# vinits5/bullet-envs

Measured on AMD Instinct MI355X. Metric: env-steps/sec (whole node), 16-link snake, 4096 envs/GPU, higher is better.
Workload: dtype f32

## Files before the change

### bullet-envs_amd/csrc/snk_pgs_v2.hpp

```cpp
#pragma once
#include "snk_contacts.hpp"
#include "snk_dynamics.hpp"
#include "snk_lds.hpp"
#include "snk_model.hpp"
#include "snk_selfcol.hpp"
#include "snk_wave.hpp"

namespace snk {


constexpr int kSlotNormal = 0;
constexpr int kSlotFric = 32;
constexpr int kSlots = 96;
constexpr int kAppMotor = 0;
constexpr int kAppNormal = 16;
constexpr int kAppFric = 80;
constexpr unsigned long long kLowMask = 0x00000000FFFFFFFFull;


struct ObsHit {
    bool hit;
    f3 P, n, dA, dB;
    float dist;
};
// ... 215 lines not shown
        f3 P = mk3(0, 0, 0), d = mk3(0, 0, 0);
        float* Mrow = motor ? L.Mm[mj] : L.stM[lane];
        if (motor) {
            k = mj + 1;
        } else {
            k = L.ccbody[ci];
            P = ld3(L.ccP[ci]);
            d = NORMAL ? (ci < L.nplane ? mk3(0.f, 0.f, 1.f) : ld3(L.obn[ci - L.nplane])) : ld3(L.cdir[L.ccds[ci]][lane >> 5]);
        }
        f3 pN = mk3(0, 0, 0), pF = mk3(0, 0, 0);
        const f3 oK = ld3(L.o[motor ? 0 : k]);
        BodyK cur = load_body_k(L, N);
#pragma unroll 4
        for (int b = N; b >= 1; b--) {
            const BodyK nxt = load_body_k(L, b > 1 ? b - 1 : 1);
            f3 ax = cur.ax;
            if (!motor && b == k) {
                pN = pN - cross(P - oK, d);
                pF = pF - d;
            }
            float u = -dot(ax, pN);
            if (motor && b == k) u += 1.0f;
            Mrow[6 + b - 1] = u;
            float t = u * cur.Dinv;
            f3 paN = pN + cur.Ua * t, paF = pF + cur.Ub * t;
            pN = paN + cross(cur.r, paF);
            pF = paF;
            cur = nxt;
        }
        f3 J0 = mk3(0, 0, 0), J1 = mk3(0, 0, 0);
        if (!motor) {
            J0 = cross(P - ld3(L.o[0]), d);
            J1 = d;
            if (k == 0) { pN = pN - J0; pF = pF - d; }
        }
        float p0[6] = {pN.x, pN.y, pN.z, pF.x, pF.y, pF.z}, a0[6];
#pragma unroll
        for (int i = 0; i < 6; i++) {
            float sum = 0.f;
#pragma unroll
            for (int j = 0; j < 6; j++) sum -= L.Inv0[6 * i + j] * p0[j];
            a0[i] = sum;
            Mrow[i] = sum;
        }
        f3 al = mk3(a0[0], a0[1], a0[2]), a = mk3(a0[3], a0[4], a0[5]);
        const float* gb = L.base() + 7;
        float den = dot(J0, al) + dot(J1, a);
        float rv = dot(J0, ld3(gb)) + dot(J1, ld3(gb + 3));
        cur = load_body_k(L, 1);
        f3 ob = ld3(L.o[1]);
        float qdb = L.qd()[0], ub = Mrow[6];
#pragma unroll 4
        for (int b = 1; b <= N; b++) {
            const int bn = b < N ? b + 1 : N;
            const BodyK nxt = load_body_k(L, bn);
            const f3 obn = ld3(L.o[bn]);
            const float qdn = L.qd()[bn - 1], un = Mrow[6 + bn - 1];
            a = a + cross(al, cur.r);
            float u = ub;
            float qdd = (u - (dot(cur.Ua, al) + dot(cur.Ub, a))) * cur.Dinv;
            f3 ax = cur.ax;
            al = al + ax * qdd;
            Mrow[6 + b - 1] = qdd;
            if (!motor) {
                float Jb = (b <= k) ? dot(ax, cross(P - ob, d)) : 0.f;
                den += Jb * qdd;
                rv += Jb * qdb;
            } else if (b == k) {
                den = qdd;
            }
            cur = nxt; ob = obn; qdb = qdn; ub = un;
        }
        float dinv = den > 1.1920929e-7f ? 1.0f / den : 0.f;
        float target;
        if (motor) {
            float cur = L.qd()[mj];
            float want = M.kp * (L.targets[mj] - L.q()[mj]) * M.inv_dt + cur + M.kd * (0.f - cur);
            target = want - cur;
        } else if (NORMAL) {
            float pen = L.ccdist[lane] + M.slop;
            float erp = M.contact_erp;
            if constexpr (LT::kERP) erp = pen > M.erp_split ? M.erp_shallow : M.erp_deep;
            target = -rv + (pen > 0.f ? -pen * M.inv_dt : -pen * erp * M.inv_dt);
        } else {
            target = -rv;
        }
        float* S = motor ? L.MmS[mj] : &L.stM[lane][22];
        S[0] = target * dinv;
        S[1] = den;
        S[2] = dinv;
        if (motor) S[3] = target;
    }
    lds_sync();
}


struct LaneK {
    int h, d;
    bool isdof;
    float m22, m24;
    float m31;
    int spoff;
    f3 oL, aL;
    int bL;
};

struct SlotRaw {
    float mval, dinv, sp, lam;
    f3 P, dir;
    int k;
    bool valid;
};
template <class LT, int KIND>
__device__ __forceinline__ SlotRaw fetch_slot(LT& L, const LaneK& K, int s, int count, int base, int nplane) {
    SlotRaw r;
    const int ci = KIND == 1 ? 2 * s + K.h : s;
    r.valid = ci < count;
    const int rs = r.valid ? ci : 0;
    const int row = KIND == 1 ? rs : (r.valid ? 32 * K.h + (s - base) : 0);
    const float* st = L.stM[row];
    const int dd = K.isdof ? K.d : 0;
    r.mval = st[dd];
    r.dinv = st[24];
    r.sp = st[22 + K.spoff];
    r.P = ld3(L.ccP[rs]);
    r.dir = KIND == 1 ? (rs < nplane ? mk3(0.f, 0.f, 1.f) : ld3(L.obn[rs - nplane])) : ld3(L.cdir[L.ccds[rs]][K.h]);
    r.k = L.ccbody[rs];
    r.lam = (KIND == 1 && r.valid) ? L.app[kAppNormal + rs] : 0.f;
    return r;
}
template <int KIND>
__device__ __forceinline__ void finish_slot(const SlotRaw& r, const LaneK& K, float sJ, float sM, float& RJ, float& RM,
                                            float& wsum) {
    float v = dot(K.aL, cross(r.P - K.oL, r.dir));
    v = K.d == 3 ? r.dir.x : (K.d == 4 ? r.dir.y : (K.d == 5 ? r.dir.z : v));
    const float jd = (K.bL <= r.k) ? v : 0.0f;
    float rj = (K.isdof ? jd * r.dinv : r.sp * K.m22) * sJ;
    float rm = (K.isdof ? r.mval : r.sp * K.m24) * sM;
    if (!r.valid) { rj = 0.f; rm = 0.f; }
    if (KIND == 1) {
        rj += K.m31 * r.lam;
        wsum += rm * r.lam;
    }
    RJ = rj;
    RM = rm;
}
struct MuScale {
    float fJ, fM, fJo, fMo;
    int nplane;
};
template <class LT, int KIND, int BASE, int DST>
__device__ __forceinline__ void load_slots8(LT& L, const LaneK& K, int count, int base, const MuScale& ms,
                                            float (&RJ)[kSlots], float (&RM)[kSlots], float& wsum) {
    SlotRaw cur = fetch_slot<LT, KIND>(L, K, BASE, count, base, ms.nplane);
#pragma unroll
    for (int i = 0; i < 8; i++) {
        SlotRaw nxt = cur;
        if (i < 7) nxt = fetch_slot<LT, KIND>(L, K, BASE + i + 1, count, base, ms.nplane);
        const bool gr = KIND == 1 || BASE + i < ms.nplane;
        finish_slot<KIND>(cur, K, KIND == 1 ? 1.0f : (gr ? ms.fJ : ms.fJo), KIND == 1 ? 1.0f : (gr ? ms.fM : ms.fMo),
                          RJ[DST + BASE + i], RM[DST + BASE + i], wsum);
        cur = nxt;
    }
}

#define SNK_REDUCE_12 \
    "v_add_f32_dpp %[t], %[t], %[t] quad_perm:[1,0,3,2] row_mask:0xf bank_mask:0xf bound_ctrl:1\n\t"
#define SNK_REDUCE_22 \
    "v_add_f32_dpp %[t], %[t], %[t] quad_perm:[2,3,0,1] row_mask:0xf bank_mask:0xf bound_ctrl:1\n\t"
#define SNK_REDUCE_345                                                                            \
    "v_add_f32_dpp %[t], %[t], %[t] row_shr:4 row_mask:0xf bank_mask:0xf bound_ctrl:1\n\t"         \
    "s_nop 1\n\t"                                                                                  \
    "v_add_f32_dpp %[t], %[t], %[t] row_shr:8 row_mask:0xf bank_mask:0xf bound_ctrl:1\n\t"         \
    "s_nop 1\n\t"                                                                                  \
    "v_add_f32_dpp %[t], %[t], %[t] row_bcast:15 row_mask:0xa bank_mask:0xf\n\t"                   \
    "s_nop 0\n\t"

#define SNK_DUO_HEAD                                     \
    "v_mul_f32 %[t], %[RJ], %[dv]\n\t"                    \
    "v_readlane_b32 %[s2], %[RJ], 31\n\t"                 \
    "v_readlane_b32 %[s3], %[RJ], 63\n\t"                 \
    SNK_REDUCE_12                                          \
    "s_nop 1\n\t"                                         \
    SNK_REDUCE_22                                          \
    "s_nop 1\n\t"                                         \
    SNK_REDUCE_345                                         \
    "v_readlane_b32 %[s0], %[t], 31\n\t"                  \
    "s_nop 1\n\t"
#define SNK_ACC3163(RJ_, T_) "v_add_f32_dpp " RJ_ ", " T_ ", " RJ_ " row_shr:15 row_mask:0xa bank_mask:0xf\n\t"
#define SNK_DUO_TAIL                                     \
    "v_cndmask_b32_e64 %[t], %[dS], %[dF], %[lowmask]\n\t" \
    "v_mul_f32 %[x], %[RM], %[t]\n\t"                     \
    "v_mul_f32 %[c2], %[RM], %[t]\n\t"                    \
    SNK_ACC3163("%[RJ]", "%[t]")                           \
    "s_nop 0\n\t"                                         \
    "v_permlane32_swap_b32 %[x], %[c2]\n\t"               \
    "v_add_f32 %[dv], %[dv], %[x]\n\t"                    \
    "v_add_f32 %[dv], %[dv], %[c2]\n\t"
template <bool RES, bool BOX>
__device__ __forceinline__ void duo_step(float& RJ, const float RM, float& dv, float HI, float E3163,
                                         unsigned long long lowmask, float& lsq) {
    float t, x, dF, dS, c2;
    float s0, s1, s2, s3;
    if (!BOX) {
        asm volatile(
            SNK_DUO_HEAD
            "v_max_f32_e64 %[dF], -%[s0], 0\n\t"
            "v_subrev_f32 %[dF], %[s2], %[dF]\n\t"
            "s_nop 0\n\t"
            "v_fmac_f32_dpp %[t], %[RJ], %[dF] row_shr:1 row_mask:0xf bank_mask:0xf bound_ctrl:1\n\t"
            "s_nop 0\n\t"
            "v_readlane_b32 %[s1], %[t], 63\n\t"
            "s_nop 1\n\t"
            "v_max_f32_e64 %[x], -%[s1], 0\n\t"
            "v_subrev_f32 %[dS], %[s3], %[x]\n\t"
            SNK_DUO_TAIL
            : [t] "=&v"(t), [x] "=&v"(x), [dF] "=&v"(dF), [dS] "=&v"(dS), [c2] "=&v"(c2), [s0] "=&s"(s0), [s1] "=&s"(s1),
              [s2] "=&s"(s2), [s3] "=&s"(s3), [RJ] "+v"(RJ), [dv] "+v"(dv)
            : [RM] "v"(RM), [lowmask] "s"(lowmask));
    } else
    asm volatile(
        SNK_DUO_HEAD
        "v_med3_f32 %[dF], -%[s0], -%[HI], %[HI]\n\t"
        "v_subrev_f32 %[dF], %[s2], %[dF]\n\t"
        "s_nop 0\n\t"
        "v_fmac_f32_dpp %[t], %[RJ], %[dF] row_shr:1 row_mask:0xf bank_mask:0xf bound_ctrl:1\n\t"
        "s_nop 0\n\t"
        "v_readlane_b32 %[s1], %[t], 63\n\t"
        "s_nop 1\n\t"
        "v_med3_f32 %[x], -%[s1], -%[HI], %[HI]\n\t"
        "v_subrev_f32 %[dS], %[s3], %[x]\n\t"
        SNK_DUO_TAIL
        : [t] "=&v"(t), [x] "=&v"(x), [dF] "=&v"(dF), [dS] "=&v"(dS), [c2] "=&v"(c2), [s0] "=&s"(s0), [s1] "=&s"(s1),
          [s2] "=&s"(s2), [s3] "=&s"(s3), [RJ] "+v"(RJ), [dv] "+v"(dv)
        : [RM] "v"(RM), [HI] "v"(HI), [lowmask] "s"(lowmask));
    if (RES) asm volatile("v_max3_f32 %[lsq], %[lsq], |%[x]|, |%[c2]|" : [lsq] "+v"(lsq) : [x] "v"(x), [c2] "v"(c2));
}

#define SNK_RED2(MODE)                                        \
    "v_add_f32_dpp %[t1], %[t1], %[t1] " MODE "\n\t"           \
    "v_add_f32_dpp %[t2], %[t2], %[t2] " MODE "\n\t"
template <bool RES>
__device__ __forceinline__ void quad_step(float& RJ1, const float RM1, float& RJ2, const float RM2, float& dv, float E3163,
                                          unsigned long long lowmask, float& lsq) {
    float t1, t2, d1, d2, d3, d4;
    float a1, a2, a3, a4, s1, s2, s3, s4;
    asm volatile(
        "v_mul_f32 %[t1], %[RJ1], %[dv]\n\t"
        "v_mul_f32 %[t2], %[RJ2], %[dv]\n\t"
        "v_readlane_b32 %[a1], %[RJ1], 31\n\t"
        SNK_RED2("quad_perm:[1,0,3,2] row_mask:0xf bank_mask:0xf bound_ctrl:1")
        "v_readlane_b32 %[a2], %[RJ1], 63\n\t"
        SNK_RED2("quad_perm:[2,3,0,1] row_mask:0xf bank_mask:0xf bound_ctrl:1")
        "v_readlane_b32 %[a3], %[RJ2], 31\n\t"
        SNK_RED2("row_shr:4 row_mask:0xf bank_mask:0xf bound_ctrl:1")
        "v_readlane_b32 %[a4], %[RJ2], 63\n\t"
        SNK_RED2("row_shr:8 row_mask:0xf bank_mask:0xf bound_ctrl:1")
        "s_nop 0\n\t"
        SNK_RED2("row_bcast:15 row_mask:0xa bank_mask:0xf")
        "v_readlane_b32 %[s1], %[t1], 31\n\t"
        "s_nop 1\n\t"
        "v_max_f32_e64 %[d1], -%[s1], 0\n\t"
        "v_subrev_f32 %[d1], %[a1], %[d1]\n\t"
        "v_fmac_f32_dpp %[t1], %[RJ1], %[d1] row_shr:1 row_mask:0xf bank_mask:0xf bound_ctrl:1\n\t"
        "v_fmac_f32_dpp %[t2], %[RJ2], %[d1] row_shr:2 row_mask:0xf bank_mask:0xf bound_ctrl:1\n\t"
        "v_readlane_b32 %[s2], %[t1], 63\n\t"
        "s_nop 1\n\t"
        "v_max_f32_e64 %[d2], -%[s2], 0\n\t"
        "v_subrev_f32 %[d2], %[a2], %[d2]\n\t"
        "v_fmac_f32_dpp %[t2], %[RJ2], %[d2] row_shr:3 row_mask:0xf bank_mask:0xf bound_ctrl:1\n\t"
        "s_nop 0\n\t"
        "v_readlane_b32 %[s3], %[t2], 31\n\t"
        "s_nop 1\n\t"
        "v_max_f32_e64 %[d3], -%[s3], 0\n\t"
        "v_subrev_f32 %[d3], %[a3], %[d3]\n\t"
        "v_fmac_f32_dpp %[t2], %[RJ2], %[d3] row_shr:1 row_mask:0xf bank_mask:0xf bound_ctrl:1\n\t"
        "s_nop 0\n\t"
        "v_readlane_b32 %[s4], %[t2], 63\n\t"
        "s_nop 1\n\t"
        "v_max_f32_e64 %[d4], -%[s4], 0\n\t"
        "v_subrev_f32 %[d4], %[a4], %[d4]\n\t"
        "v_cndmask_b32_e64 %[d1], %[d2], %[d1], %[lowmask]\n\t"
        "v_cndmask_b32_e64 %[d3], %[d4], %[d3], %[lowmask]\n\t"
        "v_mul_f32 %[t1], %[RM1], %[d1]\n\t"
        "v_mul_f32 %[t2], %[RM2], %[d3]\n\t"
        SNK_ACC3163("%[RJ1]", "%[d1]")
        SNK_ACC3163("%[RJ2]", "%[d3]")
        : [t1] "=&v"(t1), [t2] "=&v"(t2), [d1] "=&v"(d1), [d2] "=&v"(d2), [d3] "=&v"(d3), [d4] "=&v"(d4),
          [a1] "=&s"(a1), [a2] "=&s"(a2), [a3] "=&s"(a3), [a4] "=&s"(a4), [s1] "=&s"(s1), [s2] "=&s"(s2), [s3] "=&s"(s3),
          [s4] "=&s"(s4), [RJ1] "+v"(RJ1), [RJ2] "+v"(RJ2)
        : [RM1] "v"(RM1), [RM2] "v"(RM2), [dv] "v"(dv), [lowmask] "s"(lowmask));
    if (RES) asm volatile("v_max3_f32 %[lsq], %[lsq], |%[p1]|, |%[p2]|" : [lsq] "+v"(lsq) : [p1] "v"(t1), [p2] "v"(t2));
    asm volatile(
        "v_add_f32 %[p1], %[p1], %[p2]\n\t"
        "v_mov_b32 %[p2], %[p1]\n\t"
        "s_nop 1\n\t"
        "v_permlane32_swap_b32 %[p1], %[p2]\n\t"
        "v_add_f32 %[dv], %[dv], %[p1]\n\t"
        "v_add_f32 %[dv], %[dv], %[p2]\n\t"
        : [p1] "+v"(t1), [p2] "+v"(t2), [dv] "+v"(dv));
}

template <int NL, bool RES>
__device__ __forceinline__ void cone_step(float& RJ, const float RM, const float RJnorm, float& dv, float EPS,
                                          float E3163, unsigned long long lowmask, float& lsq) {
    float t, xA, xB, r2, c2;
    float s0, s1, s2, s3, s4;
    asm volatile(
        "v_mul_f32 %[t], %[RJ], %[dv]\n\t"
        "v_readlane_b32 %[s4], %[RJnorm], %[NLn]\n\t"
        "v_readlane_b32 %[s0], %[RJ], 31\n\t"
        SNK_REDUCE_12
        "v_readlane_b32 %[s2], %[RJ], 63\n\t"
        "v_mov_b32 %[xA], %[s0]\n\t"
        SNK_REDUCE_22
        "v_mov_b32 %[xB], %[s2]\n\t"
        "s_nop 0\n\t"
        SNK_REDUCE_345
        "v_readlane_b32 %[s1], %[t], 31\n\t"
        "v_readlane_b32 %[s3], %[t], 63\n\t"
        "s_nop 0\n\t"
        "v_fma_f32 %[r2], %[s1], %[s1], 1\n\t"
        "v_fma_f32 %[r2], %[s3], %[s3], %[r2]\n\t"
        "v_rsq_f32 %[r2], %[r2]\n\t"
        "s_nop 0\n\t"
        "v_mul_f32_e64 %[r2], %[s4], %[r2] clamp\n\t"
        "v_fma_f32 %[xA], %[r2], -%[s1], -%[xA]\n\t"
        "v_fma_f32 %[xB], %[r2], -%[s3], -%[xB]\n\t"
        "v_cndmask_b32_e64 %[t], %[xB], %[xA], %[lowmask]\n\t"
        "v_mul_f32 %[r2], %[RM], %[t]\n\t"
        "v_mul_f32 %[c2], %[RM], %[t]\n\t"
        SNK_ACC3163("%[RJ]", "%[t]")
        "s_nop 0\n\t"
        "v_permlane32_swap_b32 %[r2], %[c2]\n\t"
        "v_add_f32 %[dv], %[dv], %[r2]\n\t"
        "v_add_f32 %[dv], %[dv], %[c2]\n\t"
        : [t] "=&v"(t), [xA] "=&v"(xA), [xB] "=&v"(xB), [r2] "=&v"(r2), [c2] "=&v"(c2),
          [s0] "=&s"(s0), [s1] "=&s"(s1), [s2] "=&s"(s2), [s3] "=&s"(s3), [s4] "=&s"(s4), [RJ] "+v"(RJ), [dv] "+v"(dv)
        : [RM] "v"(RM), [RJnorm] "v"(RJnorm), [lowmask] "s"(lowmask),
          [NLn] "n"(NL));
    if (RES) asm volatile("v_max3_f32 %[lsq], %[lsq], |%[r2]|, |%[c2]|" : [lsq] "+v"(lsq) : [r2] "v"(r2), [c2] "v"(c2));
}

#define SNK_STR_(x) #x
#define SNK_V1(a) "v" SNK_STR_(a)
#define SNK_S1(a) "s" SNK_STR_(a)
#define SNK_VP(a, b) "v[" SNK_STR_(a) ":" SNK_STR_(b) "]"
#define SNK_SP(a, b) "s[" SNK_STR_(a) ":" SNK_STR_(b) "]"
#define SNK_CONE2_BODY_(P0, P1, P2, P3, P4, P5, Q0, Q1, Q2, Q3, Q4, Q5) \
    "v_mul_f32 %[t1], %[RJ1], %[dv]\n\t" \
    "v_mul_f32 %[t2], %[RJ2], %[dv]\n\t" \
    "v_readlane_b32 " SNK_S1(Q0) ", %[RJ1], 31\n\t" \
    "v_readlane_b32 " SNK_S1(Q1) ", %[RJ1], 63\n\t" \
    SNK_RED2("quad_perm:[1,0,3,2] row_mask:0xf bank_mask:0xf bound_ctrl:1") \
    "v_readlane_b32 " SNK_S1(Q2) ", %[RJ2], 31\n\t" \
    "v_readlane_b32 " SNK_S1(Q3) ", %[RJ2], 63\n\t" \
    SNK_RED2("quad_perm:[2,3,0,1] row_mask:0xf bank_mask:0xf bound_ctrl:1") \
    "v_readlane_b32 %[l1], %[RJn], 31\n\t" \
    "v_readlane_b32 %[l2], %[RJn], 63\n\t" \
    SNK_RED2("row_shr:4 row_mask:0xf bank_mask:0xf bound_ctrl:1") \
    "v_mov_b64 " SNK_VP(P0, P1) ", " SNK_SP(Q0, Q1) "\n\t" \
    SNK_RED2("row_shr:8 row_mask:0xf bank_mask:0xf bound_ctrl:1") \
    "v_mov_b64 " SNK_VP(P2, P3) ", " SNK_SP(Q2, Q3) "\n\t" \
    SNK_RED2("row_bcast:15 row_mask:0xa bank_mask:0xf") \
    "v_readlane_b32 " SNK_S1(Q4) ", %[t1], 31\n\t" \
    "v_readlane_b32 " SNK_S1(Q5) ", %[t1], 63\n\t" \
    "s_nop 0\n\t" \
    "v_fma_f32 " SNK_V1(P4) ", " SNK_S1(Q4) ", " SNK_S1(Q4) ", 1\n\t" \
    "v_fma_f32 " SNK_V1(P4) ", " SNK_S1(Q5) ", " SNK_S1(Q5) ", " SNK_V1(P4) "\n\t" \
    "v_rsq_f32 " SNK_V1(P4) ", " SNK_V1(P4) "\n\t" \
    "s_nop 0\n\t" \
    "v_mul_f32_e64 " SNK_V1(P4) ", %[l1], " SNK_V1(P4) " clamp\n\t" \
    "v_pk_fma_f32 " SNK_VP(P0, P1) ", " SNK_VP(P4, P5) ", " SNK_SP(Q4, Q5) ", " SNK_VP(P0, P1) " op_sel_hi:[0,1,1] neg_lo:[0,1,1] neg_hi:[0,1,1]\n\t" \
    "v_fmac_f32_dpp %[t2], %[RJ2], " SNK_V1(P0) " row_shr:1 row_mask:0xf bank_mask:0xf bound_ctrl:1\n\t" \
    "v_fmac_f32_dpp %[t2], %[RJ2], " SNK_V1(P1) " row_shr:2 row_mask:0xf bank_mask:0xf bound_ctrl:1\n\t" \
    "v_cndmask_b32_e64 " SNK_V1(P0) ", " SNK_V1(P1) ", " SNK_V1(P0) ", %[lowmask]\n\t" \
    "v_readlane_b32 " SNK_S1(Q4) ", %[t2], 31\n\t" \
    "v_readlane_b32 " SNK_S1(Q5) ", %[t2], 63\n\t" \
    "v_mul_f32 " SNK_V1(P1) ", %[RM1], " SNK_V1(P0) "\n\t" \
    SNK_ACC3163("%[RJ1]", SNK_V1(P0)) \
    "v_fma_f32 " SNK_V1(P4) ", " SNK_S1(Q4) ", " SNK_S1(Q4) ", 1\n\t" \
    "v_fma_f32 " SNK_V1(P4) ", " SNK_S1(Q5) ", " SNK_S1(Q5) ", " SNK_V1(P4) "\n\t" \
    "v_rsq_f32 " SNK_V1(P4) ", " SNK_V1(P4) "\n\t" \
    "s_nop 0\n\t" \
    "v_mul_f32_e64 " SNK_V1(P4) ", %[l2], " SNK_V1(P4) " clamp\n\t" \
    "v_pk_fma_f32 " SNK_VP(P2, P3) ", " SNK_VP(P4, P5) ", " SNK_SP(Q4, Q5) ", " SNK_VP(P2, P3) " op_sel_hi:[0,1,1] neg_lo:[0,1,1] neg_hi:[0,1,1]\n\t" \
    "v_cndmask_b32_e64 " SNK_V1(P2) ", " SNK_V1(P3) ", " SNK_V1(P2) ", %[lowmask]\n\t" \
    "v_mul_f32 " SNK_V1(P3) ", %[RM2], " SNK_V1(P2) "\n\t"
#define SNK_CONE2_TAIL_(P0, P1, P2, P3, P4, P5, Q0, Q1, Q2, Q3, Q4, Q5)                           \
    "v_add_f32 " SNK_V1(P1) ", " SNK_V1(P1) ", " SNK_V1(P3) "\n\t"           \
    "v_mov_b32 " SNK_V1(P3) ", " SNK_V1(P1) "\n\t"                 \
    SNK_ACC3163("%[RJ2]", SNK_V1(P2))                \
    "s_nop 0\n\t"                              \
    "v_permlane32_swap_b32 " SNK_V1(P1) ", " SNK_V1(P3) "\n\t"     \
    "v_add_f32 %[dv], %[dv], " SNK_V1(P1) "\n\t"         \
    "v_add_f32 %[dv], %[dv], " SNK_V1(P3) "\n\t"
#define SNK_PINS_HI 250, 251, 252, 253, 254, 255, 84, 85, 86, 87, 88, 89
#define SNK_PINS_LO 162, 163, 164, 165, 166, 167, 84, 85, 86, 87, 88, 89
#define SNK_PINS_128 122, 123, 124, 125, 126, 127, 84, 85, 86, 87, 88, 89
#define SNK_CONE2_X(M_, ...) M_(__VA_ARGS__)
#define SNK_CONE2_ASM(RESLINE, PINS, CLOB)                                                                               \
    asm volatile(SNK_CONE2_X(SNK_CONE2_BODY_, PINS) RESLINE SNK_CONE2_X(SNK_CONE2_TAIL_, PINS)                              \
                 : [t1] "=&v"(t1), [t2] "=&v"(t2), [l1] "=&s"(l1), [l2] "=&s"(l2), [RJ1] "+v"(RJ1), [RJ2] "+v"(RJ2),       \
                   [dv] "+v"(dv), [lsq] "+v"(lsq)                                                                         \
                 : [RM1] "v"(RM1), [RM2] "v"(RM2), [RJn] "v"(RJnorm), [lowmask] "s"(lowmask)                             \
                 : CLOB, "s84", "s85", "s86", "s87", "s88", "s89")
template <bool RES, int PIN = 0>
__device__ __forceinline__ void cone2_step(float& RJ1, const float RM1, float& RJ2, const float RM2, const float RJnorm,
                                           float& dv, float EPS, float E3163, unsigned long long lowmask, float& lsq) {
    float t1, t2;
    float l1, l2;
#define SNK_CLOB_HI "v250", "v251", "v252", "v253", "v254", "v255"
#define SNK_CLOB_LO "v162", "v163", "v164", "v165", "v166", "v167"
#define SNK_CLOB_128 "v122", "v123", "v124", "v125", "v126", "v127"
    if constexpr (PIN == 0) {
        if (RES) SNK_CONE2_ASM("v_max3_f32 %[lsq], %[lsq], |v251|, |v253|\n\t", SNK_PINS_HI, SNK_CLOB_HI);
        else SNK_CONE2_ASM("", SNK_PINS_HI, SNK_CLOB_HI);
    } else if constexpr (PIN == 1) {
        if (RES) SNK_CONE2_ASM("v_max3_f32 %[lsq], %[lsq], |v163|, |v165|\n\t", SNK_PINS_LO, SNK_CLOB_LO);
        else SNK_CONE2_ASM("", SNK_PINS_LO, SNK_CLOB_LO);
    } else {
        if (RES) SNK_CONE2_ASM("v_max3_f32 %[lsq], %[lsq], |v123|, |v125|\n\t", SNK_PINS_128, SNK_CLOB_128);
        else SNK_CONE2_ASM("", SNK_PINS_128, SNK_CLOB_128);
    }
}

template <int SH = 1>
__device__ __forceinline__ void cone2_coupling(const float RM1, float& RJ2, int lane) {
    const swap2 sw = half_swap(RM1, RM1);
    const float tA = half_reduce(RJ2 * sw.a);
    const float tB = half_reduce(RJ2 * sw.b);
    const float mA = __int_as_float(__builtin_amdgcn_update_dpp(0, __float_as_int(tA), 0x100 + SH, 0xf, 0xf, true));
    const float mB = __int_as_float(__builtin_amdgcn_update_dpp(0, __float_as_int(tB), 0x100 + SH + 1, 0xf, 0xf, true));
    const int d = lane & 31;
    RJ2 = d == 31 - SH ? mA : (d == 30 - SH ? mB : RJ2);
}

template <int J, bool CLAMP>
__device__ __forceinline__ float motor_step(const float RMj, float& dv, const float TARGV, float& ACCV, float PMIV) {
    float u, xs, s;
    unsigned long long sv;
    if (CLAMP) {
        asm volatile(
            "v_sub_f32 %[u], %[TARGV], %[dv]\n\t"
            "v_add_f32 %[xs], %[ACCV], %[u]\n\t"
            "v_med3_f32 %[xs], %[xs], -%[PMIV], %[PMIV]\n\t"
            "v_sub_f32 %[u], %[xs], %[ACCV]\n\t"
            "s_nop 0\n\t"
            "v_readlane_b32 %[s], %[u], %[LN]\n\t"
            "s_mov_b64 %[sv], exec\n\t"
            "s_mov_b64 exec, %[MASK]\n\t"
            "v_add_f32 %[ACCV], %[ACCV], %[u]\n\t"
            "s_mov_b64 exec, %[sv]\n\t"
            "v_fmac_f32 %[dv], %[s], %[RMj]\n\t"
            : [u] "=&v"(u), [xs] "=&v"(xs), [s] "=&s"(s), [sv] "=&s"(sv), [ACCV] "+v"(ACCV), [dv] "+v"(dv)
            : [RMj] "v"(RMj), [TARGV] "v"(TARGV), [PMIV] "v"(PMIV), [LN] "n"(6 + J), [MASK] "n"(1 << (6 + J)));
    } else {
        asm volatile(
            "v_sub_f32 %[u], %[TARGV], %[dv]\n\t"
            "s_nop 0\n\t"
            "v_readlane_b32 %[s], %[u], %[LN]\n\t"
            "s_mov_b64 %[sv], exec\n\t"
            "s_mov_b64 exec, %[MASK]\n\t"
            "v_add_f32 %[ACCV], %[ACCV], %[u]\n\t"
            "s_mov_b64 exec, %[sv]\n\t"
            "v_fmac_f32 %[dv], %[s], %[RMj]\n\t"
            : [u] "=&v"(u), [s] "=&s"(s), [sv] "=&s"(sv), [ACCV] "+v"(ACCV), [dv] "+v"(dv)
            : [RMj] "v"(RMj), [TARGV] "v"(TARGV), [LN] "n"(6 + J), [MASK] "n"(1 << (6 + J)));
        (void)xs;
    }
    return s;
}


template <bool RES, int BASE>
__device__ __forceinline__ void duos4(float (&RJ)[kSlots], float (&RM)[kSlots], float& dv, float E3163, float& lsq, int ncl) {
    quad_step<RES>(RJ[BASE], RM[BASE], RJ[BASE + 1], RM[BASE + 1], dv, E3163, kLowMask, lsq);
    if (ncl > 2 * (BASE - kSlotNormal) + 4)
        quad_step<RES>(RJ[BASE + 2], RM[BASE + 2], RJ[BASE + 3], RM[BASE + 3], dv, E3163, kLowMask, lsq);
}

template <bool RES, int G>
__device__ __forceinline__ void cones8(float (&RJ)[kSlots], float (&RM)[kSlots], float& dv, float EPS,
                                       float E3163, float& lsq, int ncl) {
#define SNK_CONE2(I)                                                                                                  \
    cone2_step<RES>(RJ[kSlotFric + 8 * G + 2 * (I)], RM[kSlotFric + 8 * G + 2 * (I)], RJ[kSlotFric + 8 * G + 2 * (I) + 1],   \
                    RM[kSlotFric + 8 * G + 2 * (I) + 1], RJ[kSlotNormal + 4 * G + (I)], dv, EPS, E3163, kLowMask, lsq);
    SNK_CONE2(0)
    SNK_CONE2(1)
    if (ncl > 8 * G + 4) {
        SNK_CONE2(2)
        SNK_CONE2(3)
    }
#undef SNK_CONE2
}

template <bool FWD, bool CLAMP, bool ALIVE, int NCO, class LT, int... K>
__device__ __forceinline__ float motors16_ordered(LT& L, const float (&RMm)[16], float& dv, const float TARGV, float& ACCV,
                                                  float PMIV, std::integer_sequence<int, K...>) {
    float res = 0.f;
    auto step = [&](auto j_c) {
        constexpr int J = decltype(j_c)::value;
        float s_ = motor_step<J, CLAMP>(RMm[J], dv, TARGV, ACCV, PMIV);
        res = fmaxf(res, fabsf(ALIVE ? s_ : s_ * (L.MmS[J][1] * L.MmS[J][2])));
    };
    (step(std::integral_constant<int, NoncontactOrder<16>::motor(FWD, K)>{}), ...);
    return res;
}
template <bool FWD, bool CLAMP, bool ALIVE, class LT>
__device__ __forceinline__ float motors16(LT& L, const float (&RMm)[16], float& dv, const float TARGV, float& ACCV,
                                          float PMIV) {
    if constexpr (LT::kNCO != 0)
        return motors16_ordered<FWD, CLAMP, ALIVE, LT::kNCO>(L, RMm, dv, TARGV, ACCV, PMIV,
                                                             std::make_integer_sequence<int, 16>{});
    float res = 0.f;
#define SNK_MOTOR(J)                                                                              \
    {                                                                                              \
        float s_ = motor_step<J, CLAMP>(RMm[J], dv, TARGV, ACCV, PMIV);                            \
        res = fmaxf(res, fabsf(ALIVE ? s_ : s_ * (L.MmS[J][1] * L.MmS[J][2])));                    \
    }
    if (FWD) {
        SNK_MOTOR(0) SNK_MOTOR(1) SNK_MOTOR(2) SNK_MOTOR(3) SNK_MOTOR(4) SNK_MOTOR(5) SNK_MOTOR(6) SNK_MOTOR(7)
        SNK_MOTOR(8) SNK_MOTOR(9) SNK_MOTOR(10) SNK_MOTOR(11) SNK_MOTOR(12) SNK_MOTOR(13) SNK_MOTOR(14) SNK_MOTOR(15)
    } else {
        SNK_MOTOR(15) SNK_MOTOR(14) SNK_MOTOR(13) SNK_MOTOR(12) SNK_MOTOR(11) SNK_MOTOR(10) SNK_MOTOR(9) SNK_MOTOR(8)
        SNK_MOTOR(7) SNK_MOTOR(6) SNK_MOTOR(5) SNK_MOTOR(4) SNK_MOTOR(3) SNK_MOTOR(2) SNK_MOTOR(1) SNK_MOTOR(0)
    }
#undef SNK_MOTOR
    return res;
}

template <bool RES>
__device__ __forceinline__ void contact_rows(float (&RJ)[kSlots], float (&RM)[kSlots], float& dv, int ncl, bool cone,
                                             float EPS, float E3163, float& lsq) {
    if (ncl > 0) duos4<RES, kSlotNormal + 0>(RJ, RM, dv, E3163, lsq, ncl);
    if (ncl > 8) duos4<RES, kSlotNormal + 4>(RJ, RM, dv, E3163, lsq, ncl);
    if (ncl > 16) duos4<RES, kSlotNormal + 8>(RJ, RM, dv, E3163, lsq, ncl);
    if (ncl > 24) duos4<RES, kSlotNormal + 12>(RJ, RM, dv, E3163, lsq, ncl);
    if (ncl > 32) duos4<RES, kSlotNormal + 16>(RJ, RM, dv, E3163, lsq, ncl);
    if (ncl > 40) duos4<RES, kSlotNormal + 20>(RJ, RM, dv, E3163, lsq, ncl);
    if (ncl > 48) duos4<RES, kSlotNormal + 24>(RJ, RM, dv, E3163, lsq, ncl);
    if (ncl > 56) duos4<RES, kSlotNormal + 28>(RJ, RM, dv, E3163, lsq, ncl);
    if (cone) {
        if (ncl > 0) cones8<RES, 0>(RJ, RM, dv, EPS, E3163, lsq, ncl);
        if (ncl > 8) cones8<RES, 1>(RJ, RM, dv, EPS, E3163, lsq, ncl);
        if (ncl > 16) cones8<RES, 2>(RJ, RM, dv, EPS, E3163, lsq, ncl);
        if (ncl > 24) cones8<RES, 3>(RJ, RM, dv, EPS, E3163, lsq, ncl);
        if (ncl > 32) cones8<RES, 4>(RJ, RM, dv, EPS, E3163, lsq, ncl);
        if (ncl > 40) cones8<RES, 5>(RJ, RM, dv, EPS, E3163, lsq, ncl);
        if (ncl > 48) cones8<RES, 6>(RJ, RM, dv, EPS, E3163, lsq, ncl);
        if (ncl > 56) cones8<RES, 7>(RJ, RM, dv, EPS, E3163, lsq, ncl);
    } else {
#pragma unroll
        for (int g = 0; g < 8; g++) {
            if (ncl > 8 * g) {
#pragma unroll
                for (int ci = 8 * g; ci < 8 * g + 8; ci++) {
                    float lim = rdlane(RJ[kSlotNormal + (ci >> 1)], (ci & 1) ? 63 : 31);
                    if (__builtin_amdgcn_readfirstlane(lim > 0.f ? 1 : 0))
                        duo_step<RES, true>(RJ[kSlotFric + ci], RM[kSlotFric + ci], dv, lim, E3163, kLowMask, lsq);
                }
            }
        }
    }
}

template <class LT>
__device__ __noinline__ void sensor_pass_v2(LT& L, const DevModel& M, const int nc, const int nlim
#ifdef SNK_PROFILE
                                            , unsigned long long* prof_t
#endif
) {
    constexpr int N = LT::kN;
    const int lane = lane_id();
    if (lane < nc) {
        const int ci = lane, k = L.ccbody[ci];
        const f3 nrm = ci < L.nplane ? mk3(0.f, 0.f, 1.f) : ld3(L.obn[ci - L.nplane]);
        f3 F = (nrm * L.app[kAppNormal + ci] +
                ld3(L.cdir[L.ccds[ci]][0]) * L.app[kAppFric + 2 * ci] +
                ld3(L.cdir[L.ccds[ci]][1]) * L.app[kAppFric + 2 * ci + 1]) * M.inv_dt;
        st3(&L.stM[ci][0], cross(ld3(L.ccP[ci]) - ld3(L.o[k]), F));
        st3(&L.stM[ci][3], F);
    }
    lds_sync();
    if (lane <= N) {
        const int b = lane;
        f3 eN = mk3(0, 0, 0), eF = mk3(0, 0, 0);
        const int c0 = b == 0 ? 0 : 2 * b - 1;
// ... 18 lines not shown
    if (lane == 0) {
        for (int i = 0; i < nlim; i++) L.tauj[L.nc_joint[i]] += L.nc_sign[i] * L.nc_app[i] * M.inv_dt;
    }
    lds_sync();
    {
        f3 wp = ld3(L.base() + 7), vp = ld3(L.base() + 10);
        if (lane == 0) { st3(L.w[0], wp); st3(L.v[0], vp); }
        for (int b = 1; b <= N; b++) {
            f3 ax = ld3(L.ax[b]), rb = ld3(L.r[b]);
            float qdb = L.qd()[b - 1];
            f3 w = wp + ax * qdb, v = vp + cross(wp, rb);
            f3 za = cross(wp, ax) * qdb, zl = cross(wp, cross(wp, rb));
            if (lane == 0) { st3(L.w[b], w); st3(L.v[b], v); st3(&L.zeta[b][0], za); st3(&L.zeta[b][3], zl); }
            wp = w; vp = v;
        }
    }
    lds_sync();
    SNK_STAMP(14)
    body_bias<LT, false>(L, M, lane);
    lds_sync();
    aba_main<LT, false>(L, M, lane);
    {
        f3 zb = mulRv(L.R[0], ld3(M.zbase));
        f3 v1 = ld3(L.base() + 10);
        float nv1 = sqrtf(dot(v1, v1));
        f3 a2 = ld3(&L.acc0[3]);
        const float fz = L.fz_park - dot(zb, a2 * M.m_root + v1 * (M.m_root * (M.lin_damp + M.lin_damp * nv1)));
        const f3 al2 = ld3(&L.acc0[0]);
        const f3 F3 = -((a2 + cross(al2, ld3(L.cw[0]))) * M.mass[0] + ld3(&L.p[0][3]));
        const float fz3 = L.fz3_park + F3.x * L.R[1][2] + F3.y * L.R[1][5] + F3.z * L.R[1][8];
        if (lane == 0) { L.fz() = fz; L.fz3() = fz3; }
    }
    SNK_STAMP(15)
}

template <class LT>
__device__ __forceinline__ void substep_v2(LT& L, const DevModel& M, int lane_in, float mu, int& iters, int& ncontacts,
                                           const SensorHint& hint, unsigned long long* __restrict__ ovf) {
    int lane = lane_in;
    constexpr int N = LT::kN;
    constexpr int ND = N + 6;
    static_assert(N == 16, "v2 is laid out for the 16-link chain");
    const float dt = M.dt;
#ifdef SNK_PROFILE
    unsigned long long prof_t[17];
#endif
    SNK_STAMP(0)
    const int nc = __builtin_amdgcn_readfirstlane(find_contacts_v2(L, M, lane, ovf));
    ncontacts = nc;
    if (nc < 0) return;
    SNK_STAMP(1)
    if (lane < N) {
        float qd = L.qd()[lane];
        L.qd_old[lane] = qd;
        L.tauj[lane] = -M.joint_damp * qd;
    }
    body_bias<LT, true>(L, M, lane);
    lds_sync();
    aba_main<LT, true>(L, M, lane);
    SNK_STAMP(2)
    {
        f3 zb = mulRv(L.R[0], ld3(M.zbase));
        f3 v_old = ld3(L.base() + 10);
        float nv0 = sqrtf(dot(v_old, v_old));
        f3 a1 = ld3(&L.acc0[3]);
        float fz1 = -dot(zb, (a1 - mk3(0.f, 0.f, M.gz)) * M.m_root + v_old * (M.m_root * (M.lin_damp + M.lin_damp * nv0)));
        const f3 al0 = ld3(&L.acc0[0]);
        const f3 F3 = -((a1 + cross(al0, ld3(L.cw[0]))) * M.mass[0] + ld3(&L.p[0][3]));
        if (lane == 0) { L.fz_park = fz1; L.fz3_park = F3.x * L.R[1][2] + F3.y * L.R[1][5] + F3.z * L.R[1][8]; }
    }
    if (lane < 6) {
        float x = L.base()[7 + lane] + L.acc0[lane] * dt;
        L.base()[7 + lane] = fminf(fmaxf(x, -M.max_vel), M.max_vel);
    } else if (lane < ND) {
        float x = L.qd()[lane - 6] + L.qdd[lane - 6] * dt;
        L.qd()[lane - 6] = fminf(fmaxf(x, -M.max_vel), M.max_vel);
    }
    lds_sync();

    SNK_STAMP(3)
    float RJ[kSlots], RM[kSlots];
    float RMm[16], TARGV;
    bool malive;
    float wsum = 0.f;
    {
        LaneK K;
        K.h = lane >> 5;
        K.d = lane & 31;
        K.isdof = K.d < ND;
        K.m22 = K.d == 22 ? -1.0f : 0.0f;
        K.m24 = K.d == 24 ? 1.0f : 0.0f;
        K.m31 = K.d == 31 ? 1.0f : 0.0f;
        K.spoff = K.d == 24 ? 1 : 0;
        K.bL = (K.d >= 6 && K.isdof) ? K.d - 5 : 0;
        K.oL = ld3(L.o[K.bL]);
        K.aL = (K.d >= 6 && K.isdof) ? ld3(L.ax[K.bL])
                                     : mk3(K.d == 0 ? 1.f : 0.f, K.d == 1 ? 1.f : 0.f, K.d == 2 ? 1.f : 0.f);
        MuScale ms;
        auto sgpr = [](float x) { return __int_as_float(__builtin_amdgcn_readfirstlane(__float_as_int(x))); };
        ms.fJ = sgpr(mu > 0.f ? 1.0f / mu : 0.f); ms.fM = sgpr(mu > 0.f ? mu : 0.f);
        const float mu_ob = fminf(M.mu_link * M.mu_obs, 10.0f);
        ms.fJo = sgpr(mu_ob > 0.f ? 1.0f / mu_ob : 0.f); ms.fMo = sgpr(mu_ob > 0.f ? mu_ob : 0.f);
        ms.nplane = __builtin_amdgcn_readfirstlane(L.nplane);
        if (nc > 64 - N || M.motors_apart) build_batch_v2<LT, 0>(L, M, lane, nc);
        SNK_STAMP(4)
#pragma unroll
        for (int s = 0; s < kSlots - kSlotFric; s++) { RJ[kSlotFric + s] = 0.f; RM[kSlotFric + s] = 0.f; }
        build_batch_v2<LT, 4>(L, M, lane, nc, 0);
        SNK_STAMP(5)
        if (nc > 0) load_slots8<LT, 4, 0, kSlotFric>(L, K, nc, 0, ms, RJ, RM, wsum);
        if (nc > 8) load_slots8<LT, 4, 8, kSlotFric>(L, K, nc, 0, ms, RJ, RM, wsum);
        if (nc > 16) load_slots8<LT, 4, 16, kSlotFric>(L, K, nc, 0, ms, RJ, RM, wsum);
        if (nc > 24) load_slots8<LT, 4, 24, kSlotFric>(L, K, nc, 0, ms, RJ, RM, wsum);
        lds_sync();
        SNK_STAMP(6)
        if (nc > 32) {
            build_batch_v2<LT, 4>(L, M, lane, nc, 32);
            SNK_STAMP(7)
            load_slots8<LT, 4, 32, kSlotFric>(L, K, nc, 32, ms, RJ, RM, wsum);
            if (nc > 40) load_slots8<LT, 4, 40, kSlotFric>(L, K, nc, 32, ms, RJ, RM, wsum);
            if (nc > 48) load_slots8<LT, 4, 48, kSlotFric>(L, K, nc, 32, ms, RJ, RM, wsum);
            if (nc > 56) load_slots8<LT, 4, 56, kSlotFric>(L, K, nc, 32, ms, RJ, RM, wsum);
            lds_sync();
        } else {
            SNK_STAMP(7)
        }
        SNK_STAMP(8)
        if (nc > 64 - N || M.motors_apart) build_batch_v2<LT, 1>(L, M, lane, nc);
        else build_batch_v2<LT, 5>(L, M, lane, nc);
        SNK_STAMP(9)
#pragma unroll
        for (int s = 0; s < kSlotFric; s++) { RJ[kSlotNormal + s] = 0.f; RM[kSlotNormal + s] = 0.f; }
        if (nc > 0) load_slots8<LT, 1, 0, kSlotNormal>(L, K, nc, 0, ms, RJ, RM, wsum);
        if (nc > 16) load_slots8<LT, 1, 8, kSlotNormal>(L, K, nc, 0, ms, RJ, RM, wsum);
        if (nc > 32) load_slots8<LT, 1, 16, kSlotNormal>(L, K, nc, 0, ms, RJ, RM, wsum);
        if (nc > 48) load_slots8<LT, 1, 24, kSlotNormal>(L, K, nc, 0, ms, RJ, RM, wsum);
#pragma unroll
        for (int j = 0; j < 16; j++) RMm[j] = K.isdof ? L.Mm[j][K.d] * L.MmS[j][2] : 0.f;
        {
            const bool mot = K.d >= 6 && K.isdof;
            const int jm = mot ? K.d - 6 : 0;
            const float dinv_m = mot ? L.MmS[jm][2] : 0.f;
            TARGV = (mot && dinv_m > 0.f) ? L.MmS[jm][3] : 0.f;
            malive = __all(!mot || dinv_m > 0.f) != 0;
        }
        lds_sync();
    }

    SNK_STAMP(10)
    {
#pragma unroll
        for (int g = 0; g < 8; g++) {
            if (nc > 8 * g) {
#pragma unroll
                for (int i = 0; i < 4; i++) {
                    const int s = kSlotNormal + 4 * g + i;
                    swap2 sw = half_swap(RM[s], RM[s]);
                    float t = half_reduce(RJ[s] * sw.a);
                    RJ[s] = wrlane(RJ[s], rdlane(t, 63), 62);
                }
#pragma unroll
                for (int i = 0; i < 2; i++) {
                    const int s = kSlotNormal + 4 * g + 2 * i;
                    cone2_coupling<2>(RM[s], RJ[s + 1], lane);
                }
            }
        }
        if (M.cone == 0) {
#pragma unroll
            for (int g = 0; g < 8; g++) {
                if (nc > 8 * g) {
#pragma unroll
                    for (int i = 0; i < 8; i++) {
                        const int s = kSlotFric + 8 * g + i;
                        swap2 sw = half_swap(RM[s], RM[s]);
                        float t = half_reduce(RJ[s] * sw.a);
                        RJ[s] = wrlane(RJ[s], rdlane(t, 63), 62);
                    }
                }
            }
        } else {
#pragma unroll
            for (int g = 0; g < 8; g++) {
                if (nc > 8 * g) {
#pragma unroll
                    for (int i = 0; i < 4; i++) {
                        const int s = kSlotFric + 8 * g + 2 * i;
                        cone2_coupling(RM[s], RJ[s + 1], lane);
                    }
                }
            }
        }
    }

    SNK_STAMP(11)
    int nlim = 0;
    {
        bool viol = false;
        float sgn = 0.f, pen = 0.f;
        if (lane < N) {
            float qj = L.q()[lane];
            float plo = qj - M.jlo, phi = M.jhi - qj;
            if (plo <= 0.f) { viol = true; sgn = 1.f; pen = plo; }
            else if (phi <= 0.f) { viol = true; sgn = -1.f; pen = phi; }
        }
        unsigned long long bal = __ballot(viol);
        nlim = __builtin_amdgcn_readfirstlane(__popcll(bal));
        if (viol) {
            unsigned long long before = (1ull << lane) - 1ull;
            if constexpr (LT::kNCO != 0) before = NoncontactOrder<N>::tab.below[lane];
            int idx = __popcll(bal & before);
            float den = L.Mm[lane][6 + lane];
            float dinv = den > 1.1920929e-7f ? 1.0f / den : 0.f;
            float rel = sgn * L.qd()[lane];
            L.nc_joint[idx] = lane; L.nc_sign[idx] = sgn;
            L.nc_rhs[idx] = (-rel + (-pen) * M.limit_erp * M.inv_dt) * dinv;
            L.nc_dinv[idx] = dinv; L.nc_den[idx] = den;
            L.nc_lo[idx] = 0.f; L.nc_hi[idx] = M.limit_max; L.nc_app[idx] = 0.f;
        }
        if (nlim) lds_sync();
    }

    SNK_STAMP(12)
    __builtin_amdgcn_s_setprio(3);
    float dv;
    {
        const int d = lane & 31;
        dv = d == 22 ? 1.0f : (d == 31 ? -1.0f : 0.0f);
        {
            const swap2 sw = half_swap(wsum, wsum);
            dv += sw.a + sw.b;
        }
        const float E3163 = d == 31 ? 1.0f : 0.0f;
        const float EPS = 1e-30f;
        const float mi = M.max_motor_imp;
        const bool mclamp = mi < 1e30f;
        float ACCV = 0.f;
        const float thr = __int_as_float(__builtin_amdgcn_readfirstlane(__float_as_int(sqrtf(M.resid_thr))));
        const int n_iter = M.n_iter;
        const bool cone = M.cone != 0;
        int it = 0;
#pragma unroll
        for (int s2 = 0; s2 < kSlots; s2++) asm volatile("" : "+v"(RJ[s2]), "+v"(RM[s2]));
#pragma unroll
        for (int j2 = 0; j2 < 16; j2++) asm volatile("" : "+v"(RMm[j2]));
        for (; it < n_iter; it++) {
            int exceeded = 0;
            int ncl = nc;
            asm volatile("" : "+s"(ncl));
#pragma unroll
            for (int s2 = 0; s2 < kSlots; s2++) asm volatile("" : "+v"(RJ[s2]), "+v"(RM[s2]));
            auto limit_rows = [&](bool fwd) {
                for (int jj = 0; jj < nlim; jj++) {
                    const int idx = fwd ? jj : nlim - 1 - jj;
                    const int j = __builtin_amdgcn_readfirstlane(L.nc_joint[idx]);
                    const float sg = L.nc_sign[idx];
                    float un = sg * rdlane(dv, 6 + j);
                    float a0 = L.nc_app[idx];
                    float dI = L.nc_rhs[idx] - un * L.nc_dinv[idx];
                    float sum = fminf(fmaxf(a0 + dI, L.nc_lo[idx]), L.nc_hi[idx]);
                    dI = sum - a0;
                    L.nc_app[idx] = sum;
                    float mv = (d < ND) ? L.Mm[j][d] : 0.f;
                    dv += sg * mv * dI;
                    if (__builtin_amdgcn_readfirstlane(fabsf(dI * L.nc_den[idx]) > thr ? 1 : 0)) exceeded = 1;
                }
            };
            float mres;
            auto pmiv = [&]() {
                const bool mot = d >= 6 && d < ND;
                const float dinv_m = mot ? L.MmS[mot ? d - 6 : 0][2] : 0.f;
                return (dinv_m > 0.f) ? mi / dinv_m : 1e30f;
            };
#define SNK_MOTORS(FWD)                                                                             \
    mres = malive ? (mclamp ? motors16<FWD, true, true>(L, RMm, dv, TARGV, ACCV, pmiv())             \
                            : motors16<FWD, false, true>(L, RMm, dv, TARGV, ACCV, 0.f))              \
                  : (mclamp ? motors16<FWD, true, false>(L, RMm, dv, TARGV, ACCV, pmiv())            \
                            : motors16<FWD, false, false>(L, RMm, dv, TARGV, ACCV, 0.f));
            if constexpr (LT::kNCO == 0) {
                if (it & 1) {
                    limit_rows(true);
                    SNK_MOTORS(true)
                } else {
                    SNK_MOTORS(false)
                    limit_rows(false);
                }
            } else {
                if (it & 1) {
                    SNK_MOTORS(true)
                    limit_rows(true);
                } else {
                    limit_rows(false);
                    SNK_MOTORS(false)
                }
            }
#undef SNK_MOTORS
            if (__builtin_amdgcn_readfirstlane(mres > thr ? 1 : 0)) exceeded = 1;
            {
                float l_ = 0.f;
                contact_rows<true>(RJ, RM, dv, ncl, cone, EPS, E3163, l_);
                float m = fmaxf(rdlane(l_, 24), rdlane(l_, 56));
                if (__builtin_amdgcn_readfirstlane(m > thr ? 1 : 0)) exceeded = 1;
            }
            if (!exceeded || it >= n_iter - 1) { it++; break; }
        }
        iters = it;
        lane = lane_id();
        if ((lane & 31) == 31) {
            const int h = lane >> 5;
#pragma unroll
            for (int s = 0; s < kSlotFric; s++) L.app[kAppNormal + 2 * s + h] = RJ[kSlotNormal + s];
            const int npl = L.nplane;
            const float mu_ob = fminf(M.mu_link * M.mu_obs, 10.0f);
#pragma unroll
            for (int s = 0; s < kSlots - kSlotFric; s++) L.app[kAppFric + 2 * s + h] = RJ[kSlotFric + s] * (s < npl ? mu : mu_ob);
        }
        if (lane >= 6 && lane < ND) L.app[kAppMotor + lane - 6] = ACCV * L.MmS[lane - 6][2];
    }
    lds_sync();
    if (M.contact_model == 1 && lane < 2 * N) {
        int idx = L.cylbase[lane];
        const int mask = L.cylkeep[lane];
#pragma unroll
        for (int j = 0; j < 4; j++)
            if ((mask >> j) & 1) L.mfl[6 * j + 5][lane] = L.app[kAppNormal + idx++];
    }

    SNK_STAMP(13)
    __builtin_amdgcn_s_setprio(0);
    const bool sensor = sensor_pass_needed(L, M, lane, dv, hint);
    L.stM[lane][20] = dv;
#ifdef SNK_PROFILE
    prof_t[14] = prof_t[13]; prof_t[15] = prof_t[13];
    if (sensor && lane == 0) atomicAdd(ovf + 2, 1ull);
#endif
    if (sensor) {
#ifdef SNK_PROFILE
        sensor_pass_v2(L, M, nc, nlim, prof_t);
#else
        sensor_pass_v2(L, M, nc, nlim);
#endif
    }
// ... 47 lines not shown
```

Before: 374,500.

## Batch coupling reductions into interleaved asm and skip dead slot-loads

```diff
diff --git a/bullet-envs_amd/csrc/snk_pgs_v2.hpp b/bullet-envs_amd/csrc/snk_pgs_v2.hpp
--- a/bullet-envs_amd/csrc/snk_pgs_v2.hpp
+++ b/bullet-envs_amd/csrc/snk_pgs_v2.hpp
@@ -391,11 +391,14 @@
 template <class LT, int KIND, int BASE, int DST>
 __device__ __forceinline__ void load_slots8(LT& L, const LaneK& K, int count, int base, const MuScale& ms,
                                             float (&RJ)[kSlots], float (&RM)[kSlots], float& wsum) {
+    const int live = KIND == 1 ? (count + 1) >> 1 : count;
+    const bool second = live > BASE + 4;
     SlotRaw cur = fetch_slot<LT, KIND>(L, K, BASE, count, base, ms.nplane);
 #pragma unroll
     for (int i = 0; i < 8; i++) {
+        if (i == 4 && !second) break;
         SlotRaw nxt = cur;
-        if (i < 7) nxt = fetch_slot<LT, KIND>(L, K, BASE + i + 1, count, base, ms.nplane);
+        if (i < 7 && (i != 3 || second)) nxt = fetch_slot<LT, KIND>(L, K, BASE + i + 1, count, base, ms.nplane);
         const bool gr = KIND == 1 || BASE + i < ms.nplane;
         finish_slot<KIND>(cur, K, KIND == 1 ? 1.0f : (gr ? ms.fJ : ms.fJo), KIND == 1 ? 1.0f : (gr ? ms.fM : ms.fMo),
                           RJ[DST + BASE + i], RM[DST + BASE + i], wsum);
@@ -664,15 +667,101 @@
     }
 }
 
+#define SNK_CPL_QP1 "quad_perm:[1,0,3,2] row_mask:0xf bank_mask:0xf bound_ctrl:1"
+#define SNK_CPL_STEP4(T0, T1, T2, T3, MODE)                      \
+    "v_add_f32_dpp " T0 ", " T0 ", " T0 " " MODE "\n\t"            \
+    "v_add_f32_dpp " T1 ", " T1 ", " T1 " " MODE "\n\t"            \
+    "v_add_f32_dpp " T2 ", " T2 ", " T2 " " MODE "\n\t"            \
+    "v_add_f32_dpp " T3 ", " T3 ", " T3 " " MODE "\n\t"
+#define SNK_CPL_REDUCE4(T0, X0, Y0, T1, X1, Y1, T2, X2, Y2, T3, X3, Y3)                  \
+    "v_mov_b32_dpp " T0 ", " T0 " " SNK_CPL_QP1 "\n\t"                                    \
+    "v_mov_b32_dpp " T1 ", " T1 " " SNK_CPL_QP1 "\n\t"                                    \
+    "v_mov_b32_dpp " T2 ", " T2 " " SNK_CPL_QP1 "\n\t"                                    \
+    "v_mov_b32_dpp " T3 ", " T3 " " SNK_CPL_QP1 "\n\t"                                    \
+    "v_fmac_f32 " T0 ", " X0 ", " Y0 "\n\t"                                               \
+    "v_fmac_f32 " T1 ", " X1 ", " Y1 "\n\t"                                               \
+    "v_fmac_f32 " T2 ", " X2 ", " Y2 "\n\t"                                               \
+    "v_fmac_f32 " T3 ", " X3 ", " Y3 "\n\t"                                               \
+    SNK_CPL_STEP4(T0, T1, T2, T3, "quad_perm:[2,3,0,1] row_mask:0xf bank_mask:0xf bound_ctrl:1") \
+    SNK_CPL_STEP4(T0, T1, T2, T3, "row_shr:4 row_mask:0xf bank_mask:0xf bound_ctrl:1")      \
+    SNK_CPL_STEP4(T0, T1, T2, T3, "row_shr:8 row_mask:0xf bank_mask:0xf bound_ctrl:1")      \
+    SNK_CPL_STEP4(T0, T1, T2, T3, "row_bcast:15 row_mask:0xa bank_mask:0xf bound_ctrl:1")
+
+__device__ __forceinline__ void duo_coupling4(const float RM0, float& RJ0, const float RM1, float& RJ1, const float RM2,
+                                              float& RJ2, const float RM3, float& RJ3) {
+    float a0, a1, a2, a3, t0, t1, t2, t3;
+    float s0, s1, s2, s3;
+    asm volatile(
+        "v_mov_b32 %[a0], %[RM0]\n\t"
+        "v_mov_b32 %[t0], %[RM0]\n\t"
+        "v_mov_b32 %[a1], %[RM1]\n\t"
+        "v_mov_b32 %[t1], %[RM1]\n\t"
+        "v_mov_b32 %[a2], %[RM2]\n\t"
+        "v_mov_b32 %[t2], %[RM2]\n\t"
+        "v_mov_b32 %[a3], %[RM3]\n\t"
+        "v_mov_b32 %[t3], %[RM3]\n\t"
+        "v_permlane32_swap_b32 %[a0], %[t0]\n\t"
+        "v_permlane32_swap_b32 %[a1], %[t1]\n\t"
+        "v_permlane32_swap_b32 %[a2], %[t2]\n\t"
+        "v_permlane32_swap_b32 %[a3], %[t3]\n\t"
+        "v_mul_f32 %[t0], %[RJ0], %[a0]\n\t"
+        "v_mul_f32 %[t1], %[RJ1], %[a1]\n\t"
+        "v_mul_f32 %[t2], %[RJ2], %[a2]\n\t"
+        "v_mul_f32 %[t3], %[RJ3], %[a3]\n\t"
+        SNK_CPL_REDUCE4("%[t0]", "%[RJ0]", "%[a0]", "%[t1]", "%[RJ1]", "%[a1]", "%[t2]", "%[RJ2]", "%[a2]", "%[t3]", "%[RJ3]",
+                        "%[a3]")
+        "v_readlane_b32 %[s0], %[t0], 63\n\t"
+        "v_readlane_b32 %[s1], %[t1], 63\n\t"
+        "v_readlane_b32 %[s2], %[t2], 63\n\t"
+        "v_readlane_b32 %[s3], %[t3], 63\n\t"
+        "v_writelane_b32 %[RJ0], %[s0], 62\n\t"
+        "v_writelane_b32 %[RJ1], %[s1], 62\n\t"
+        "v_writelane_b32 %[RJ2], %[s2], 62\n\t"
+        "v_writelane_b32 %[RJ3], %[s3], 62\n\t"
+        : [a0] "=&v"(a0), [a1] "=&v"(a1), [a2] "=&v"(a2), [a3] "=&v"(a3), [t0] "=&v"(t0), [t1] "=&v"(t1), [t2] "=&v"(t2),
+          [t3] "=&v"(t3), [s0] "=&s"(s0), [s1] "=&s"(s1), [s2] "=&s"(s2), [s3] "=&s"(s3), [RJ0] "+v"(RJ0), [RJ1] "+v"(RJ1),
+          [RJ2] "+v"(RJ2), [RJ3] "+v"(RJ3)
+        : [RM0] "v"(RM0), [RM1] "v"(RM1), [RM2] "v"(RM2), [RM3] "v"(RM3));
+}
+
 template <int SH = 1>
-__device__ __forceinline__ void cone2_coupling(const float RM1, float& RJ2, int lane) {
-    const swap2 sw = half_swap(RM1, RM1);
-    const float tA = half_reduce(RJ2 * sw.a);
-    const float tB = half_reduce(RJ2 * sw.b);
-    const float mA = __int_as_float(__builtin_amdgcn_update_dpp(0, __float_as_int(tA), 0x100 + SH, 0xf, 0xf, true));
-    const float mB = __int_as_float(__builtin_amdgcn_update_dpp(0, __float_as_int(tB), 0x100 + SH + 1, 0xf, 0xf, true));
-    const int d = lane & 31;
-    RJ2 = d == 31 - SH ? mA : (d == 30 - SH ? mB : RJ2);
+__device__ __forceinline__ void cone2_coupling2(const float RMP, float& RJP, const float RMQ, float& RJQ) {
+    float aP, bP, aQ, bQ, tAP, tBP, tAQ, tBQ;
+    float s0, s1, s2, s3;
+    asm volatile(
+        "v_mov_b32 %[aP], %[RMP]\n\t"
+        "v_mov_b32 %[bP], %[RMP]\n\t"
+        "v_mov_b32 %[aQ], %[RMQ]\n\t"
+        "v_mov_b32 %[bQ], %[RMQ]\n\t"
+        "s_nop 0\n\t"
+        "v_permlane32_swap_b32 %[aP], %[bP]\n\t"
+        "v_permlane32_swap_b32 %[aQ], %[bQ]\n\t"
+        "v_mul_f32 %[tAP], %[RJP], %[aP]\n\t"
+        "v_mul_f32 %[tBP], %[RJP], %[bP]\n\t"
+        "v_mul_f32 %[tAQ], %[RJQ], %[aQ]\n\t"
+        "v_mul_f32 %[tBQ], %[RJQ], %[bQ]\n\t"
+        SNK_CPL_REDUCE4("%[tAP]", "%[RJP]", "%[aP]", "%[tBP]", "%[RJP]", "%[bP]", "%[tAQ]", "%[RJQ]", "%[aQ]", "%[tBQ]",
+                        "%[RJQ]", "%[bQ]")
+        "v_readlane_b32 %[s0], %[tAP], 31\n\t"
+        "v_readlane_b32 %[s1], %[tAP], 63\n\t"
+        "v_readlane_b32 %[s2], %[tBP], 31\n\t"
+        "v_readlane_b32 %[s3], %[tBP], 63\n\t"
+        "v_writelane_b32 %[RJP], %[s0], %[LA]\n\t"
+        "v_writelane_b32 %[RJP], %[s1], %[HA]\n\t"
+        "v_writelane_b32 %[RJP], %[s2], %[LB]\n\t"
+        "v_writelane_b32 %[RJP], %[s3], %[HB]\n\t"
+        "v_readlane_b32 %[s0], %[tAQ], 31\n\t"
+        "v_readlane_b32 %[s1], %[tAQ], 63\n\t"
+        "v_readlane_b32 %[s2], %[tBQ], 31\n\t"
+        "v_readlane_b32 %[s3], %[tBQ], 63\n\t"
+        "v_writelane_b32 %[RJQ], %[s0], %[LA]\n\t"
+        "v_writelane_b32 %[RJQ], %[s1], %[HA]\n\t"
+        "v_writelane_b32 %[RJQ], %[s2], %[LB]\n\t"
+        "v_writelane_b32 %[RJQ], %[s3], %[HB]\n\t"
+        : [aP] "=&v"(aP), [bP] "=&v"(bP), [aQ] "=&v"(aQ), [bQ] "=&v"(bQ), [tAP] "=&v"(tAP), [tBP] "=&v"(tBP),
+          [tAQ] "=&v"(tAQ), [tBQ] "=&v"(tBQ), [s0] "=&s"(s0), [s1] "=&s"(s1), [s2] "=&s"(s2), [s3] "=&s"(s3),
+          [RJP] "+v"(RJP), [RJQ] "+v"(RJQ)
+        : [RMP] "v"(RMP), [RMQ] "v"(RMQ), [LA] "n"(31 - SH), [HA] "n"(63 - SH), [LB] "n"(30 - SH), [HB] "n"(62 - SH));
 }
 
 template <int J, bool CLAMP>
@@ -997,42 +1086,27 @@
 #pragma unroll
         for (int g = 0; g < 8; g++) {
             if (nc > 8 * g) {
-#pragma unroll
-                for (int i = 0; i < 4; i++) {
-                    const int s = kSlotNormal + 4 * g + i;
-                    swap2 sw = half_swap(RM[s], RM[s]);
-                    float t = half_reduce(RJ[s] * sw.a);
-                    RJ[s] = wrlane(RJ[s], rdlane(t, 63), 62);
-                }
-#pragma unroll
-                for (int i = 0; i < 2; i++) {
-                    const int s = kSlotNormal + 4 * g + 2 * i;
-                    cone2_coupling<2>(RM[s], RJ[s + 1], lane);
-                }
+                const int s = kSlotNormal + 4 * g;
+                duo_coupling4(RM[s], RJ[s], RM[s + 1], RJ[s + 1], RM[s + 2], RJ[s + 2], RM[s + 3], RJ[s + 3]);
+                cone2_coupling2<2>(RM[s], RJ[s + 1], RM[s + 2], RJ[s + 3]);
             }
         }
         if (M.cone == 0) {
 #pragma unroll
             for (int g = 0; g < 8; g++) {
                 if (nc > 8 * g) {
-#pragma unroll
-                    for (int i = 0; i < 8; i++) {
-                        const int s = kSlotFric + 8 * g + i;
-                        swap2 sw = half_swap(RM[s], RM[s]);
-                        float t = half_reduce(RJ[s] * sw.a);
-                        RJ[s] = wrlane(RJ[s], rdlane(t, 63), 62);
-                    }
+                    const int s = kSlotFric + 8 * g;
+                    duo_coupling4(RM[s], RJ[s], RM[s + 1], RJ[s + 1], RM[s + 2], RJ[s + 2], RM[s + 3], RJ[s + 3]);
+                    duo_coupling4(RM[s + 4], RJ[s + 4], RM[s + 5], RJ[s + 5], RM[s + 6], RJ[s + 6], RM[s + 7], RJ[s + 7]);
                 }
             }
         } else {
 #pragma unroll
             for (int g = 0; g < 8; g++) {
                 if (nc > 8 * g) {
-#pragma unroll
-                    for (int i = 0; i < 4; i++) {
-                        const int s = kSlotFric + 8 * g + 2 * i;
-                        cone2_coupling(RM[s], RJ[s + 1], lane);
-                    }
+                    const int s = kSlotFric + 8 * g;
+                    cone2_coupling2(RM[s], RJ[s + 1], RM[s + 2], RJ[s + 3]);
+                    cone2_coupling2(RM[s + 4], RJ[s + 5], RM[s + 6], RJ[s + 7]);
                 }
             }
         }
```

Result: no change. 376,600, median of 6 (+0.6%).
